# DarianNwankwo/Rollout-Bayesian-Optimization

Hardware: NVIDIA B200
Metric: rollout trajectories/sec (value+grad) (higher is better)
Workload: dtype f64

## Files before the change

### rollout-bayesian-optimization_b200/csrc/rollout_kernel.cu

```cuda
#include "rbo_kernel.cuh"

#ifndef RBO_VGLOB
#define RBO_VGLOB 0
#endif
#if RBO_VGLOB
#define RBO_ROW_UNROLL _Pragma("unroll 4")
#else
#define RBO_ROW_UNROLL _Pragma("unroll 2")
#endif
#if RBO_VGLOB
#define RBO_KERNEL_NAME rbo_rollout_kernel_largen
#define g_phase_cycles g_phase_cycles_largen
#define g_aux_cycles g_aux_cycles_largen
#define g_tr_cycles g_tr_cycles_largen
#else
#define RBO_KERNEL_NAME rbo_rollout_kernel
#endif

namespace rbo {

#ifdef RBO_PHASE_TIMERS
__device__ unsigned long long g_phase_cycles[16];
__device__ unsigned long long g_aux_cycles[16];
__device__ unsigned long long g_tr_cycles[16];
#define TR_T(v) long long v = clock64()
#define TR_ADD(i, t0, t1) do { if ((threadIdx.x & 31) == 0) atomicAdd(&g_tr_cycles[i], (unsigned long long)((t1) - (t0))); } while (0)
#define AUX_T(v) long long v = clock64()
#define AUX_ADD(i, t0) do { } while (0)
#define PT_DECL long long pt_t0 = clock64()
#define PT_MARK(i) do { if (threadIdx.x == 0) { long long t1_ = clock64(); atomicAdd(&g_phase_cycles[i], (unsigned long long)(t1_ - pt_t0)); pt_t0 = t1_; } } while (0)
#else
#define PT_DECL
#define PT_MARK(i)
#define AUX_T(v)
#define AUX_ADD(i, t0)
#define TR_T(v)
#define TR_ADD(i, t0, t1)
#endif

namespace {

enum { I_M = 0, I_NACT = 1, I_TSTATUS = 2, I_BEST = 3, I_EVALS = 4, I_T = 5, I_CASE = 6, I_NEXT = 7, I_ARR = 64 };
constexpr unsigned FULL = 0xffffffffu;
#ifndef RBO_SPIN_CAP
#define RBO_SPIN_CAP (1u << 28)
#endif

__device__ __forceinline__ double warp_sum(double v) {
#pragma unroll
  for (int off = 16; off > 0; off >>= 1) v += __shfl_xor_sync(FULL, v, off);
  return v;
}
__device__ __forceinline__ double warp_max(double v) {
#pragma unroll
  for (int off = 16; off > 0; off >>= 1) v = fmax(v, __shfl_xor_sync(FULL, v, off));
  return v;
}
__device__ __forceinline__ double warp_min(double v) {
#pragma unroll
  for (int off = 16; off > 0; off >>= 1) v = fmin(v, __shfl_xor_sync(FULL, v, off));
  return v;
}
__device__ __forceinline__ double warp_max_nonneg(double v) {
  const unsigned hi = (unsigned)__double2hiint(v), lo = (unsigned)__double2loint(v);
  const unsigned mh = __reduce_max_sync(FULL, hi);
  const unsigned ml = __reduce_max_sync(FULL, hi == mh ? lo : 0u);
  return __hiloint2double((int)mh, (int)ml);
}
__device__ __forceinline__ int tri_idx(int p, int q, int n) { return p * n - (p * (p - 1)) / 2 + (q - p); }

__device__ __forceinline__ void dmma(double& c0, double& c1, double a, double b) {
  asm volatile("mma.sync.aligned.m8n8k4.row.col.f64.f64.f64.f64 {%0,%1}, {%2}, {%3}, {%0,%1};" : "+d"(c0), "+d"(c1) : "d"(a), "d"(b));
}
__device__ __forceinline__ void c_to_b(double c0, double c1, int g, int tg, double& b0, double& b1) {
    const int s0 = tg * 4 + (g >> 1), s1 = s0 + 16;
    const double a0 = __shfl_sync(FULL, c0, s0), a1 = __shfl_sync(FULL, c1, s0);
    const double e0 = __shfl_sync(FULL, c0, s1), e1 = __shfl_sync(FULL, c1, s1);
    b0 = (g & 1) ? a1 : a0; b1 = (g & 1) ? e1 : e0;
  }
__device__ __forceinline__ void fan_wbot(const double* V, const double* Fp, int RP, int N8, int cB, int nfan, int g, int tg, double& w0, double& w1) {
    const double t0 = (tg < nfan) ? V[(size_t)(N8 + tg) * RP + cB] : 0.0;
    const double t1 = (tg + 4 < nfan) ? V[(size_t)(N8 + tg + 4) * RP + cB] : 0.0;
    w0 = 0.0; w1 = 0.0;
    dmma(w0, w1, Fp[(size_t)(N8 + g) * 8 + tg], t0);
    dmma(w0, w1, Fp[(size_t)(N8 + g) * 8 + 4 + tg], t1);
    if (g >= nfan) { w0 = 0.0; w1 = 0.0; }
  }

__device__ __noinline__ void bwd_direct(double* V, const double* Fp, const int* colidx, const double* Lbf, int RP, int N8, int nb, int ncols, int nfan, int warp, int lane, double* scratch = nullptr) {
    const unsigned FULL = 0xffffffffu;
    const int g = lane >> 2, tg = lane & 3;
    const int ngroups = (ncols + 7) >> 3, ncls = (nb + 1) >> 1, tpg = ncls * 4;
    auto cols = [&](int group, int& cB, int& c0, int& c1, bool& v0, bool& v1) {
      const int i0 = 8 * group, first = colidx[i0];
      cB = (i0 + g < ncols) ? colidx[i0 + g] : first;
      v0 = i0 + 2 * tg < ncols; v1 = i0 + 2 * tg + 1 < ncols;
      c0 = v0 ? colidx[i0 + 2 * tg] : first; c1 = v1 ? colidx[i0 + 2 * tg + 1] : first;
    };
    if (nfan > 0) {
      const int ntile = N8 >> 3;
      for (int task = warp; task < ngroups * ntile; task += RBO_NWARPS) {
        const int group = task / ntile, i0 = 8 * (task - group * ntile);
        int cB, c0, c1; bool v0, v1;
        cols(group, cB, c0, c1, v0, v1);
        double w0, w1, b0, b1;
        fan_wbot(V, Fp, RP, N8, cB, nfan, g, tg, w0, w1);
        c_to_b(w0, w1, g, tg, b0, b1);
        double* vr = V + (size_t)(i0 + g) * RP;
        double x0 = vr[c0], x1 = vr[c1];
        dmma(x0, x1, Fp[(size_t)(i0 + g) * 8 + tg], -b0);
        dmma(x0, x1, Fp[(size_t)(i0 + g) * 8 + 4 + tg], -b1);
        __syncwarp();
        if (v0) vr[c0] = x0;
        if (v1) vr[c1] = x1;
      }
      __syncthreads();
      for (int group = warp; group < ngroups; group += RBO_NWARPS) {
        int cB, c0, c1; bool v0, v1;
        cols(group, cB, c0, c1, v0, v1);
        double w0, w1;
        fan_wbot(V, Fp, RP, N8, cB, nfan, g, tg, w0, w1);
        __syncwarp();
        if (v0) V[(size_t)(N8 + g) * RP + c0] = w0;
        if (v1) V[(size_t)(N8 + g) * RP + c1] = w1;
      }
    }
#if RBO_VGLOB
    {
      const int ntask = ngroups * ncls;
      __syncthreads();
      for (int task = warp; task < ntask; task += RBO_NWARPS) {
        const int group = task / ncls, cls = task - group * ncls;
        int cB, c0, c1; bool v0, v1;
        cols(group, cB, c0, c1, v0, v1);
        const int rp4 = 4 * RP, rp8 = 8 * RP;
        for (int hh = 0; hh < 2; ++hh) {
          const int ib = hh ? nb - 1 - cls : cls, rb = RBO_BR * ib;
          if (hh && ib == cls) continue;
          const int nc = nb - ib, chunk0 = nb * ib - ib * (ib - 1) / 2;
          const int nq = min(4, (N8 - rb + 7) >> 3);
          const double2* ap = reinterpret_cast<const double2*>(Lbf) + (size_t)chunk0 * 512 + lane;
          const double* vd = V + (size_t)(rb + tg) * RP + cB;
          double acc[4][4];
#pragma unroll
          for (int q = 0; q < 4; ++q) { acc[q][0] = acc[q][1] = acc[q][2] = acc[q][3] = 0.0; }
          for (int cc = 0; cc < nc; ++cc) {
            const double* v = (cc < nc - 1) ? vd + (size_t)(RBO_BR + RBO_CHUNK_K * cc) * RP : vd;
            double bv[8];
#pragma unroll
            for (int pp = 0; pp < 4; ++pp) { bv[2 * pp] = v[pp * rp8]; bv[2 * pp + 1] = v[pp * rp8 + rp4]; }
            const double2* ac = ap + (size_t)512 * cc;
#pragma unroll
            for (int q = 0; q < 4; ++q) {
              if (q < nq) {
                double2 A[4];
#pragma unroll
                for (int pp = 0; pp < 4; ++pp) A[pp] = __ldg(ac + 128 * q + 32 * pp);
#pragma unroll
                for (int pp = 0; pp < 4; ++pp) {
                  dmma(acc[q][0], acc[q][1], A[pp].x, bv[2 * pp]);
                  dmma(acc[q][2], acc[q][3], A[pp].y, bv[2 * pp + 1]);
                }
              }
            }
          }
#pragma unroll
          for (int q = 0; q < 4; ++q) {
            const int row = rb + 8 * q + g;
            if (q < nq && row < N8) {
              double* o = scratch + ((size_t)group * N8 + row) * 8 + 2 * tg;
              o[0] = acc[q][0] + acc[q][2]; o[1] = acc[q][1] + acc[q][3];
            }
          }
        }
      }
      __syncthreads();
      for (int idx = threadIdx.x; idx < ngroups * N8 * 8; idx += RBO_THREADS) {
        const int group = idx / (N8 * 8), r2 = idx - group * N8 * 8, row = r2 >> 3, cc = r2 & 7;
        if (8 * group + cc < ncols) V[(size_t)row * RP + colidx[8 * group + cc]] = scratch[idx];
      }
    }
#else
    const int gpb = RBO_NWARPS / tpg;
    for (int gb = 0; gb < ngroups; gb += gpb) {
      const int group = gb + warp / tpg, rem = warp % tpg, cls = rem >> 2, rq = rem & 3;
      const bool wact = warp < gpb * tpg && group < ngroups;
      int cB = 0, c0 = 0, c1 = 0; bool v0 = false, v1 = false;
      if (wact) cols(group, cB, c0, c1, v0, v1);
      double acc[2][2] = {{0.0, 0.0}, {0.0, 0.0}};
      const int rp4 = 4 * RP, rp8 = 8 * RP;
      __syncthreads();
#pragma unroll
      for (int hh = 0; hh < 2; ++hh) {
        const int ib = hh ? nb - 1 - cls : cls, rb = RBO_BR * ib;
        if (!wact || (hh && ib == cls) || rb + 8 * rq >= N8) continue;
// ... 817 lines not shown
      double* fv = V + cB;
      const int fp = tg;

      AUX_T(tf0_);
      if (!FWD && nfan > 0 && wact) {
        if (rq == 0) {
          double t[8], wb[8];
#pragma unroll
          for (int r = 0; r < 8; ++r) t[r] = (r < nfan) ? fv[(size_t)(N8 + r) * RP] : 0.0;
          __syncwarp();
#pragma unroll
          for (int r = 0; r < 8; ++r) {
            double s = 0.0;
#pragma unroll
            for (int kk = 0; kk < 8; ++kk) s = fma(Fp[(size_t)(N8 + r) * 8 + kk], t[kk], s);
            wb[r] = (r < nfan) ? s : 0.0;
          }
          if (vB && fp == 0) {
#pragma unroll
            for (int r = 0; r < 8; ++r) fv[(size_t)(N8 + r) * RP] = wb[r];
          }
          for (int i = fp; i < N8; i += 4) {
            const double* f = Fp + (size_t)i * 8;
            double s = 0.0;
#pragma unroll
            for (int r = 0; r < 8; ++r) s = fma(f[r], wb[r], s);
            if (vB) fv[(size_t)i * RP] -= s;
          }
        }
        group_sync(NRQ, gl);
      }

      AUX_ADD(1, tf0_);
      AUX_T(tc0_);
      double c[MTW][2];
#pragma unroll
      for (int mt = 0; mt < MTW; ++mt) { c[mt][0] = 0.0; c[mt][1] = 0.0; }
      const int rofs = 8 * MTW * rq;
      for (int i = 0; i < nb; ++i) {
        const int ib = FWD ? nb - 1 - i : i, nc = FWD ? ib + 1 : nb - ib, rb = RBO_BR * ib;
        for (int cc = 0; cc < nc; ++cc, ++q) {
#ifdef RBO_PHASE_TIMERS
          long long tw0 = clock64();
#endif
          full_wait(q);
#ifdef RBO_PHASE_TIMERS
          if (tid == 0) atomicAdd(&g_phase_cycles[FWD ? 12 : 13], (unsigned long long)(clock64() - tw0));
#endif
          const double* buf = stage + (size_t)(q % RBO_NSTAGE) * RBO_CHUNK_K * RBO_LP + rofs;
          AUX_T(tm0_);
          if (wact) {
            const int nt = (N8 - rb - rofs + 7) >> 3;
            if (cc < nc - 1) {
              const int krow0 = (FWD ? 0 : rb + RBO_BR) + cc * RBO_CHUNK_K;
              mma_chunk<MTW>(buf, V + (size_t)krow0 * RP, cB, g, tg, c, nt);
            } else {
              mma_chunk<MTW>(buf, V + (size_t)rb * RP, cB, g, tg, c, nt);
              AUX_T(td0_);
              group_sync(NRQ, gl);
#pragma unroll
              for (int mt = 0; mt < MTW; ++mt) {
                const int row = rb + rofs + 8 * mt + g;
                if (row < N8) {
                  if (v0) V[(size_t)row * RP + c0] = c[mt][0];
                  if (v1) V[(size_t)row * RP + c1] = c[mt][1];
                }
                c[mt][0] = 0.0; c[mt][1] = 0.0;
              }
              asm volatile("" ::: "memory");
              AUX_ADD(4, td0_);
            }
          }
          __syncwarp();
          AUX_ADD(3, tm0_);
          if (lane == 0) empty_arrive(q);
        }
      }

      AUX_ADD(2, tc0_);
      if (FWD && nfan > 0 && wact && NRQ > 1) group_sync(NRQ, gl);
      if (FWD && nfan > 0 && wact && rq == 0) {
        double a0[2] = {0.0, 0.0}, a1[2] = {0.0, 0.0};
        const double* fa = Fp + (size_t)tg * 8 + g;
        const double* vb = V + (size_t)tg * RP + cB;
        const int nkt = N8 >> 2;
#pragma unroll 2
        for (int kt = 0; kt < nkt; kt += 2) {
          dmma(a0[0], a1[0], fa[(size_t)(4 * kt) * 8], vb[(size_t)(4 * kt) * RP]);
          dmma(a0[1], a1[1], fa[(size_t)(4 * kt + 4) * 8], vb[(size_t)(4 * kt + 4) * RP]);
        }
        const double s0 = a0[0] + a0[1], s1 = a1[0] + a1[1];
        double* vr = V + (size_t)(N8 + g) * RP;
        const double t0 = (g < nfan) ? vr[c0] - s0 : 0.0, t1 = (g < nfan) ? vr[c1] - s1 : 0.0;
        double b0, b1, r0 = 0.0, r1 = 0.0;
        c_to_b(t0, t1, g, tg, b0, b1);
        dmma(r0, r1, Fp[(size_t)(N8 + tg) * 8 + g], b0);
        dmma(r0, r1, Fp[(size_t)(N8 + tg + 4) * 8 + g], b1);
        if (g >= nfan) { r0 = 0.0; r1 = 0.0; }
        __syncwarp();
        if (v0) vr[c0] = r0;
        if (v1) vr[c1] = r1;
        __syncwarp();
      }
    }
    qglob = q;
  }

  __device__ void assemble_warp(int sl, int aidx, int np, int RSpre, const double* p1, int nout1, int RS1, const double* pg, int noutg, int goff, int gld,
                                int RSg, int RShc, int RShw, double fstar, double* Href ) {
    const int d = P.d, dd = d * d, q1 = d + 1, T2 = d * (d + 1) / 2;
    const double* ppre = sm + pl.ppre; const double* phess = sm + pl.phess;
    const int nout_pre = np * q1;
    double* dmu = sm + pl.sdmu + sl * d; double* dsig = sm + pl.sdsig + sl * d; double* ga = sm + pl.sga + sl * d;
    double* Ht = sm + pl.sHt + sl * dd; double* gh = sm + pl.sgh + sl * 8;
    auto pre = [&](int e) {
      double s = 0.0;
      if (RSpre < 0) { for (int r = 0; r < RS1; ++r) s += p1[(size_t)r * nout1 + e * (-RSpre) + q1]; }
      else for (int r = 0; r < RSpre; ++r) s += ppre[(size_t)r * nout_pre + aidx * q1 + e];
      return s;
    };
    auto one = [&](int e) { double s = 0.0; for (int r = 0; r < RS1; ++r) s += p1[(size_t)r * nout1 + e]; return s; };
    auto gramf = [&](int p, int q) { double s = 0.0; for (int r = 0; r < RSg; ++r) s += pg[(size_t)r * noutg + goff + p * gld + q]; return s; };
    auto hes = [&](int which, int e) { double s = 0.0; const int RS = which ? RShw : RShc; for (int r = 0; r < RS; ++r) s += phess[((size_t)(r * np + aidx) * 2 + which) * (T2 + 1) + e]; return s; };
    const double mu = pre(0);
    const double var = P.k0 - one(0);
    const double sigma = sqrt(var), isg = 1.0 / sigma;
    const GPart g = rule_eval(P.rule_id, P.sigma_tol, mu, sigma, P.theta1, fstar);
    bool fin = isfinite(g.g);
    for (int p = lane; p < d; p += 32) {
      double m = pre(1 + p), sg = -one(1 + p) * isg;
      double a = g.g_mu * m + g.g_sig * sg;
      dmu[p] = m; dsig[p] = sg; ga[p] = a;
      fin = fin && isfinite(a);
    }
    __syncwarp();
    const double bC = hes(0, T2), bW = hes(1, T2);
    for (int e = lane; e < T2; e += 32) {
      const int pq = tbld[e], p = pq & 0xff, q = pq >> 8;
      double gram = gramf(p, q), hc = hes(0, e), hw = hes(1, e);
      if (p == q) { hc += bC; hw += bW; }
      double hs = (-dsig[p] * dsig[q] - gram - hw) * isg;
      double href = g.g_mumu * dmu[p] * dmu[q] + g.g_mu * hc + g.g_sigsig * dsig[p] * dsig[q] + g.g_sig * hs;
      double htrue = href + g.g_musig * (dmu[p] * dsig[q] + dsig[p] * dmu[q]);
      if (Href) { Href[p * d + q] = href; Href[q * d + p] = href; }
      Ht[p * d + q] = -htrue; Ht[q * d + p] = -htrue;
      fin = fin && isfinite(htrue);
    }
    fin = __all_sync(FULL, fin);
    if (lane == 0) {
      gh[0] = g.g; gh[1] = g.g_mu; gh[2] = g.g_sig; gh[3] = g.g_muth; gh[4] = g.g_sigth; gh[5] = sigma; gh[6] = mu;
      gh[7] = fin ? 1.0 : 0.0;
    }
    __syncwarp();
  }

  __device__ bool chol_warp(double* A, int n) const {
    for (int j = 0; j < n; ++j) {
      double t = 0.0;
      if (lane >= j && lane < n) {
        t = A[lane * n + j];
        for (int k = 0; k < j; ++k) t = fma(-A[lane * n + k], A[j * n + k], t);
      }
      const double tj = __shfl_sync(FULL, t, j);
      if (!(tj > 0.0) || !isfinite(tj)) return false;
      const double inv = rsqrt(tj);
      if (lane == j) A[j * n + j] = inv;
      else if (lane > j && lane < n) A[lane * n + j] = t * inv;
      __syncwarp();
    }
    return true;
  }

  __device__ bool slot_logic_warp(int sl, bool single = false) {
    const int d = P.d, dd = d * d;
    const rbo_solver_opts& o = P.so;
    double* x = sm + pl.sx + sl * d; double* xt = sm + pl.sxt + sl * d; double* g = sm + pl.sg + sl * d;
    double* H = sm + pl.sH + sl * dd;
    double* Ht = sm + pl.sHt + sl * dd;
    double* A = Ht;
    const double* ga = sm + pl.sga + sl * d; const double* gh = sm + pl.sgh + sl * 8;
    int* fr = sfr + 32 * sl;
    TR_T(l0_);
    double f = (sm + pl.sf)[sl], Delta = (sm + pl.slam)[sl], pred = (sm + pl.spred)[sl], alpha = (sm + pl.shs)[sl];
    int iters = siter[sl], tries = stry[sl], flg = sflag[sl];
    double sn = (sm + pl.ssn)[sl];
    const double at = gh[0];
    bool fin = gh[7] != 0.0;
    const int ph = phase[sl];
    __syncwarp();
    auto store = [&](int status, bool keep) {
      if (lane == 0) {
        (sm + pl.sf)[sl] = f; (sm + pl.slam)[sl] = Delta; (sm + pl.spred)[sl] = pred; (sm + pl.shs)[sl] = alpha; (sm + pl.ssn)[sl] = sn;
        siter[sl] = iters; stry[sl] = tries; sflag[sl] = flg;
        if (!keep) sstat[sl] = status;
        phase[sl] = keep ? 1 : 2;
      }
      __syncwarp();
      return keep;
    };
    const double* lb = sm + pl.sbnd; const double* ub = lb + d;
    const int T2 = d * (d + 1) / 2;
    auto accept_state = [&](double fnew) {
      alpha = at;
      f = fnew;
      if (flg & 1) {
        const double ia = 1.0 / at;
        for (int a = lane; a < d; a += 32) { x[a] = xt[a]; g[a] = -ga[a] * ia; }
        __syncwarp();
        for (int e = lane; e < T2; e += 32) {
          const int pq = tbld[e], p = pq & 0xff, q = pq >> 8;
          const double hv = Ht[p * d + q] * ia + g[p] * g[q];
          H[p * d + q] = hv; H[q * d + p] = hv;
        }
      } else {
        for (int a = lane; a < d; a += 32) { x[a] = xt[a]; g[a] = -ga[a]; }
        for (int i = lane; i < dd; i += 32) H[i] = Ht[i];
      }
      __syncwarp();
    };
    if (lane == 0) sevals[sl] += 1;
    bool fresh;
    if (ph == 0) {
      if (!fin) {
        for (int a = lane; a < d; a += 32) x[a] = xt[a];
        alpha = nan("");
        return store(RBO_SOLVE_NAN, false);
      }
      flg = (P.rule_id != RBO_RULE_LCB && at > 0.0) ? 1 : 0;
      accept_state((flg & 1) ? -log(at) : -at);
      if (single) return store(RBO_SOLVE_CONVERGED, false);
      double wmax = 0.0;
      for (int a = 0; a < d; ++a) wmax = fmax(wmax, P.ubs[a] - P.lbs[a]);
      Delta = fmin(o.delta0_box * wmax, o.delta0_ell * P.kern.th[0]);
      iters = 0; tries = 0;
      fresh = true;
    } else {
      fin = fin && (!(flg & 1) || at > 0.0);
      const double ft = fin ? ((flg & 1) ? -log(at) : -at) : 0.0;
      const double rho = fin ? (f - ft) / pred : -1.0;
      if (fin && rho >= o.eta) {
        accept_state(ft);
        if (rho > 0.75 && (flg & 2) && sn >= 0.8 * Delta) {
          double dm2 = 0.0;
          for (int a = 0; a < d; ++a) { const double wd = P.ubs[a] - P.lbs[a]; dm2 = fma(wd, wd, dm2); }
          Delta = fmin(2.0 * Delta, sqrt(dm2));
        } else if (rho < 0.25) Delta = 0.25 * sn;
        tries = 0;
        iters += 1;
        if (iters >= o.maxit) return store(RBO_SOLVE_MAXIT, false);
        fresh = true;
      } else {
        Delta = 0.25 * fmin(Delta, sn);
        tries += 1;
        if (tries >= o.maxtry) return store(RBO_SOLVE_STALLED, false);
        fresh = false;
      }
    }
    const bool in = lane < d;
    const double xa = in ? x[lane] : 0.0, gg = in ? g[lane] : 0.0;
    const double lba = in ? lb[lane] : 0.0, uba = in ? ub[lane] : 0.0;
    const bool act = in && ((xa <= lba && gg > 0.0) || (xa >= uba && gg < 0.0));
    const bool isfree = in && !act;
    const unsigned fmask = __ballot_sync(FULL, isfree);
    const int nfree = __popc(fmask);
    if (isfree) fr[__popc(fmask & ((1u << lane) - 1u))] = lane;
    double pg = warp_max_nonneg(isfree ? fabs(gg) : 0.0);
    if (flg & 1) pg *= alpha;
    __syncwarp();
    if (fresh && pg <= o.gtol * fmax(1.0, fabs(alpha))) return store(RBO_SOLVE_CONVERGED, false);
    const int myc = lane < nfree ? fr[lane] : 0;
    const double xmax = warp_max_nonneg(fabs(xa));
    for (;;) {
      double* yv = sm + pl.sdmu + sl * d;
      TR_T(l1_); TR_ADD(1, l0_, l1_); TR_ADD(0, 0, 1);
      const bool hit = (nfree >= 2 && nfree <= 16) ? tr_step16(H, g, fr, nfree, d, Delta, sm + pl.sdsig + sl * d, sm + pl.sga + sl * d, yv)
                                                  : tr_step_warp(H, g, fr, nfree, d, Delta, A, yv);
      const double t = lane < nfree ? yv[lane] : 0.0;
      TR_T(l2_); TR_ADD(2, l1_, l2_);
      if (in) xt[lane] = xa;
      __syncwarp();
      if (lane < nfree) xt[myc] = fmin(fmax(x[myc] + t, lb[myc]), ub[myc]);
      __syncwarp();
      const double sa = in ? xt[lane] - xa : 0.0;
      const double smax = warp_max_nonneg(fabs(sa));
      if (smax <= o.xtol * fmax(1.0, xmax)) { sn = sqrt(warp_sum(sa * sa)); return store(RBO_SOLVE_STEP_TINY, false); }
      if (in) yv[lane] = sa;
      __syncwarp();
      double hsv = 0.0;
      if (in) {
        const double* Hr = H + lane * d;
        if ((d & 1) == 0) {
          double h1 = 0.0;
          for (int b = 0; b < d; b += 2) {
            const double2 hh = *reinterpret_cast<const double2*>(Hr + b), ss = *reinterpret_cast<const double2*>(yv + b);
            hsv = fma(hh.x, ss.x, hsv); h1 = fma(hh.y, ss.y, h1);
          }
          hsv += h1;
        } else for (int b = 0; b < d; ++b) hsv = fma(Hr[b], yv[b], hsv);
      }
      double r0 = sa * sa, r1 = gg * sa, r2 = sa * hsv;
#pragma unroll
      for (int off = 16; off > 0; off >>= 1) {
        r0 += __shfl_xor_sync(FULL, r0, off); r1 += __shfl_xor_sync(FULL, r1, off); r2 += __shfl_xor_sync(FULL, r2, off);
      }
      sn = sqrt(r0);
      const double gs = r1, sHs = r2;
      const double pr = -(gs + 0.5 * sHs);
      if (!(pr > 0.0)) {
        Delta = 0.25 * fmin(Delta, sn);
        tries += 1;
        if (tries >= o.maxtry) return store(RBO_SOLVE_STALLED, false);
        continue;
      }
      const bool pred_tiny = pr <= o.pred_tol * fmax(1.0, fabs(f));
      if (!hit && (pred_tiny || smax <= o.stol * fmax(1.0, xmax))) {
        for (int a = lane; a < d; a += 32) x[a] = xt[a];
        alpha = (flg & 1) ? alpha * exp(pr) : alpha + pr;
        return store(RBO_SOLVE_FINAL_STEP, false);
      }
      if (pred_tiny) return store(RBO_SOLVE_PRED_TINY, false);
      pred = pr;
      flg = (flg & 1) | (hit ? 2 : 0);
      TR_T(l3_); TR_ADD(3, l2_, l3_);
      return store(0, true);
    }
  }

  __device__ void load_start(int sl, int sid) {
    const int d = P.d;
    phase[sl] = 0; sstat[sl] = RBO_SOLVE_MAXIT; siter[sl] = 0; stry[sl] = 0; sevals[sl] = 0; sstart[sl] = sid; sflag[sl] = 0;
    for (int a = 0; a < d; ++a) {
      double v = __ldg(P.starts + (size_t)sid * d + a);
      (sm + pl.sxt)[sl * d + a] = fmin(fmax(v, P.lbs[a]), P.ubs[a]);
    }
  }

  __device__ void multistart(size_t tape_off, bool single = false, bool first = false) {
    const int d = P.d, W = P.W, q1 = d + 1;
    __syncthreads();
    const unsigned short* evsrc = first ? evfirst : evprev;
    for (int i = tid; i < P.S; i += RBO_THREADS) {
      const unsigned e = evsrc[i];
      int r = 0;
      for (int j = 0; j < P.S; ++j) { const unsigned ej = evsrc[j]; r += (ej > e || (ej == e && j < i)) ? 1 : 0; }
      sorder[r] = (unsigned short)i;
    }
    __syncthreads();
    if (tid == 0) {
      si[I_BEST] = -1; si[I_EVALS] = 0; misc[0] = 0.0;
      const int n0 = single ? 1 : min(W, P.S);
      for (int i = 0; i < n0; ++i) { alist[i] = i; load_start(i, single ? i : (int)sorder[i]); }
      if (single) for (int a = 0; a < d; ++a) (sm + pl.sxt)[a] = bestx[a];
      si[I_NACT] = n0; si[I_NEXT] = single ? P.S : n0;
    }
    __syncthreads();
    int nact = si[I_NACT];
    PT_DECL;
    const long long round_cap = (long long)P.S * (P.so.maxit + 2) * (P.so.maxtry + 2);
    long long rounds_ = 0;
    while (nact > 0) {
      if (++rounds_ > round_cap) { if (tid == 0) P.work_counter[2] = 1; break; }
      auto pt = [&](int s) { return (const double*)(sm + pl.sxt + alist[s] * d); };
      auto cb = [&](int s) { return alist[s] * P.CS; };
      PT_MARK(9);
      fill_columns(nact, pt, cb);
      for (int i = tid; i < nact * q1; i += RBO_THREADS) { int s = i / q1; colidx[i] = alist[s] * P.CS + (i - s * q1); }
      const int nbq = nblk16(q1);
      __syncthreads();
      PT_MARK(0);
      tri_solve<true>(nact * q1, nf);
      const int q2 = q1 + 1;
      for (int s = tid; s < nact; s += RBO_THREADS) set_item(s, alist[s] * P.CS, q1, alist[s] * P.CS, q2, s * q1 * q2, UCOL);
      __syncthreads();
      PT_MARK(2);
      const int RS1 = choose_rs(nact * nbq * nblk16(q2)), RSg = RS1;
      colprod(nact, nact * q1 * q2, sm + pl.ppost, RS1);
      for (int i = tid; i < nact; i += RBO_THREADS) colidx[i] = alist[i] * P.CS;
      __syncthreads();
      PT_MARK(3);
      tri_solve<false>(nact, nf);
      __syncthreads();
      PT_MARK(4);
      const int nbd = nblk16(d);
      const int RShw = max(1, min(P.RSh, RBO_NWARPS / (nact * (nbd * (nbd + 1) / 2)))), RShc = RShw;
      hess_sums<3>(nact, pt, cb, cb, RShw);
      __syncthreads();
      PT_MARK(5);
      {
        const int n1 = nact * q1 * q2, nh = nact * 2 * (d * (d + 1) / 2 + 1);
        double* pp = sm + pl.ppost; double* ph = sm + pl.phess;
        if (RS1 > 1) for (int i = tid; i < n1; i += RBO_THREADS) { double a_ = pp[i]; for (int r = 1; r < RS1; ++r) a_ += pp[(size_t)r * n1 + i]; pp[i] = a_; }
        if (RShw > 1) for (int i = tid; i < nh; i += RBO_THREADS) { double a_ = ph[i]; for (int r = 1; r < RShw; ++r) a_ += ph[(size_t)r * nh + i]; ph[i] = a_; }
        __syncthreads();
      }
      for (int s = warp; s < nact; s += RBO_NWARPS) {
        const int sl = alist[s];
        assemble_warp(sl, s, nact, -q2, sm + pl.ppost + s * q1 * q2, nact * q1 * q2, 1, sm + pl.ppost, nact * q1 * q2, s * q1 * q2 + q2 + 1, q2, 1, 1, 1, misc[1], single ? sm + pl.sHref : nullptr);
#ifdef RBO_PHASE_TIMERS
        long long ta_ = clock64();
        if (tid == 0) atomicAdd(&g_phase_cycles[8], (unsigned long long)(ta_ - pt_t0));
#endif
        slot_logic_warp(sl, single);
#ifdef RBO_PHASE_TIMERS
        if (tid == 0) atomicAdd(&g_phase_cycles[14], (unsigned long long)(clock64() - ta_));
        if (lane == 0) { long long dt_ = clock64() - ta_; int b_ = (int)(dt_ / 4000); atomicAdd(&g_aux_cycles[b_ > 15 ? 15 : b_], 1ull); }
#endif
      }
      __syncthreads();
      PT_MARK(6);
      if (tid == 0) {
        int na2 = 0;
        for (int i = 0; i < nact; ++i) {
          const int sl = alist[i];
          if (phase[sl] == 1) { alist[na2++] = sl; continue; }
          const int sid = sstart[sl];
          const double f = -(sm + pl.shs)[sl];
          const double* x = sm + pl.sx + sl * d;
          bool bad = !isfinite(f);
          for (int a = 0; a < d; ++a) bad = bad || isnan(x[a]);
          si[I_EVALS] += sevals[sl];
          if (!single) { evprev[sid] = (unsigned short)min(sevals[sl], 65535); if (first) evfirst[sid] = evprev[sid]; }
          if (P.start_status && !single) P.start_status[tape_off + sid] = sstat[sl];
          if (P.start_iters && !single) P.start_iters[tape_off + sid] = siter[sl];
          if (!bad && (si[I_BEST] < 0 || f < misc[0] || (f == misc[0] && sid < si[I_BEST]))) {
            si[I_BEST] = sid; misc[0] = f;
            for (int a = 0; a < d; ++a) bestx[a] = x[a];
          }
          if (si[I_NEXT] < P.S) { load_start(sl, (int)sorder[si[I_NEXT]]); si[I_NEXT] += 1; alist[na2++] = sl; }
        }
        si[I_NACT] = na2;
      }
      __syncthreads();
      PT_MARK(7);
#ifdef RBO_PHASE_TIMERS
      if (tid == 0) atomicAdd(&g_phase_cycles[15], 1ull);
#endif
      nact = si[I_NACT];
    }
    if (tid == 0 && si[I_BEST] < 0) {
      if (si[I_TSTATUS] == RBO_TRAJ_OK) si[I_TSTATUS] = RBO_TRAJ_ALL_STARTS_NAN;
      for (int a = 0; a < d; ++a) bestx[a] = nan("");
    }
    __syncthreads();
  }
};

}

__global__ void __launch_bounds__(RBO_THREADS, 1) RBO_KERNEL_NAME(const __grid_constant__ DevProblem P) {
  extern __shared__ __align__(128) double smem[];
  K k(P, smem);
  const int tid = k.tid, d = P.d, N8 = P.N8, NR = P.NR, RP = P.RP, h = P.h, q1 = d + 1;
  double* bestx = k.bestx;
  double* misc = k.misc;
  int* si = k.si;
  k.build_tables();
  for (int i = tid; i < 2 * d; i += RBO_THREADS) smem[P.pl.sbnd + i] = i < d ? P.lbs[i] : P.ubs[i - d];
  for (int i = tid; i < P.S; i += RBO_THREADS) { k.evprev[i] = 0; k.evfirst[i] = 0; }
  k.pipe_init();
  for (int i = tid; i < NR * RP; i += RBO_THREADS) k.V[i] = 0.0;
  if (P.xsm) for (int i = tid; i < d * N8; i += RBO_THREADS) k.Xs[(i / N8) * P.XP + (i % N8)] = __ldg(P.Xb + i);
  __syncthreads();

  for (;;) {
    __syncthreads();
    if (tid == 0) {
      const int i = atomicAdd(P.work_counter, 1);
      si[I_M] = (i < P.M) ? (P.order ? P.order[i] : i) : P.M;
    }
    __syncthreads();
    const int m = si[I_M];
    if (m >= P.M) break;
#define RBO_MS (m % P.Ms)
#define RBO_MB (m / P.Ms)

    for (int i = tid; i < (N8 + RBO_MAXFAN) * 8; i += RBO_THREADS) k.Fp[i] = 0.0;
    for (int i = tid; i < 64; i += RBO_THREADS) k.G[i] = ((i >> 3) == (i & 7)) ? 1.0 : 0.0;
    for (int i = tid; i < NR; i += RBO_THREADS) { double c = (i < N8) ? __ldg(P.c0 + i) : 0.0; k.cst[i] = c; k.V[(size_t)i * RP + k.CCOL] = c; }
    for (int i = tid; i < NR; i += RBO_THREADS) { double u0 = (i < N8) ? __ldg(P.u0 + i) : 0.0; k.u[i] = u0; k.V[(size_t)i * RP + k.UCOL] = u0; }
    __syncthreads();
    if (tid < 8) k.Fp[(size_t)(N8 + tid) * 8 + tid] = 1.0;
    if (tid == 0) { misc[1] = P.ymin_base; si[I_TSTATUS] = RBO_TRAJ_OK; }
    k.nf = 0;
    __syncthreads();

    const bool myopic = (P.flags & RBO_FLAG_MYOPIC_INTERNAL) != 0;
    for (int step = myopic ? 1 : 0; step <= (myopic ? 1 : h); ++step) {
      if (step == 0) {
        if (tid < d) bestx[tid] = P.x0_batch ? __ldg(P.x0_batch + (size_t)RBO_MB * d + tid) : P.x0[tid];
        __syncthreads();
      } else {
        for (int pass = 0; pass < 2; ++pass) {
          const bool single = pass == 1;
          if (single && (myopic || !(P.flags & RBO_FLAG_TAPE_EX))) break;
          if (!single && !myopic && (P.flags & RBO_FLAG_TEACHER_FORCED)) {
            if (tid < d) bestx[tid] = (P.flags & RBO_FLAG_REPLAY_TAPE) ? P.xs[((size_t)m * (h + 1) + step) * d + tid] : P.x_forced[((size_t)RBO_MS * h + (step - 1)) * d + tid];
            if (tid == 0) { si[I_EVALS] = 0; misc[0] = nan(""); }
          } else {
            if (single) __syncthreads();
            k.multistart(single ? 0 : (myopic ? (size_t)m * P.S : ((size_t)m * h + (step - 1)) * P.S), single, !single && step == 1);
          }
          __syncthreads();
          if (!single) {
            if (!myopic && tid == 0) {
              if (P.n_evals) P.n_evals[(size_t)m * h + step - 1] = si[I_EVALS];
              if (P.alphas) P.alphas[(size_t)m * h + step - 1] = -misc[0];
            }
          } else {
            const size_t o = (size_t)m * h + step - 1;
            const double* gh = smem + k.pl.sgh;
            if (tid == 0) { P.t_mu[o] = gh[6]; P.t_sigma[o] = gh[5]; if (P.alphas) P.alphas[o] = gh[0]; }
            for (int i = tid; i < d; i += RBO_THREADS) { P.t_dmu[o * d + i] = (smem + k.pl.sdmu)[i]; P.t_dsigma[o * d + i] = (smem + k.pl.sdsig)[i]; }
            for (int i = tid; i < d * d; i += RBO_THREADS) P.t_Halpha[o * d * d + i] = (smem + k.pl.sHref)[i];
            __syncthreads();
          }
        }
      }
      if (myopic) {
        if (tid < d) P.xs[(size_t)m * d + tid] = bestx[tid];
        if (tid == 0) {
          P.values[m] = -misc[0];
          if (P.n_evals) P.n_evals[m] = si[I_EVALS];
          if (P.status) P.status[m] = si[I_TSTATUS];
          if (P.best_index) P.best_index[m] = si[I_BEST];
          if (P.grad_case) P.grad_case[m] = 0;
        }
        break;
      }

      {
        PT_DECL;
        auto pt = [&](int) { return (const double*)bestx; };
        auto cb0 = [&](int) { return 0; };
        k.fill_columns(1, pt, cb0);
        k.set_column(k.UCOL, k.u);
        for (int i = tid; i < q1; i += RBO_THREADS) k.colidx[i] = i;
        if (tid == 0) k.set_item(0, 0, q1, k.CCOL, 1, 0);
        __syncthreads();
        const int nbq = K::nblk16(q1);
        const int RSpre = k.choose_rs(nbq);
        k.colprod(1, q1, smem + k.pl.ppre, RSpre);
        __syncthreads();
        k.tri_solve<true>(q1, k.nf);
        if (tid == 0) { k.set_item(0, 0, q1, 0, q1, 0); k.set_item(1, 0, 1, k.UCOL, 1, q1 * q1); }
        __syncthreads();
        const int nsg = q1 * q1 + 1;
        const int RSpost = k.choose_rs(nbq * nbq + 1);
        k.colprod(2, nsg, smem + k.pl.ppost, RSpost);
        __syncthreads();
        double* Sg = misc + 8;
        for (int e = tid; e < nsg; e += RBO_THREADS) {
          double acc = 0.0;
          for (int r = 0; r < RSpost; ++r) acc += (smem + k.pl.ppost)[(size_t)r * nsg + e];
          if (e < q1 * q1) {
            const int p = e / q1, q = e - p * q1;
            const double dk = (p == q) ? (p == 0 ? P.k0 : -P.d2k0) : 0.0;
            if (p <= q) { Sg[p * q1 + q] = dk - acc; Sg[q * q1 + p] = dk - acc; }
            if (p == 0) misc[8 + q1 * q1 + q1 + q] = acc;
            if (e == 0) misc[4] = acc;
          } else misc[5] = acc;
        }
        if (tid < q1) {
          double acc = 0.0;
          for (int r = 0; r < RSpre; ++r) acc += (smem + k.pl.ppre)[(size_t)r * q1 + tid];
          misc[8 + q1 * q1 + tid] = acc;
        }
        __syncthreads();
        if (tid == 0) {
          const int r = k.nf;
          const double* dmu = misc + 8 + q1 * q1;
          double yv;
          if (P.flags & RBO_FLAG_GAUSS_HERMITE) {
            const double* raw = misc + 8 + q1 * q1 + q1;
            const double var = P.k0 - raw[0];
            if (!(var >= 0.0) && si[I_TSTATUS] == RBO_TRAJ_OK) si[I_TSTATUS] = RBO_TRAJ_NEG_VARIANCE;
            const double sigma = sqrt(var), node = __ldg(P.gh_nodes + (size_t)RBO_MS * P.gh_depth + step), s2n = 1.4142135623730951 * node;
            yv = dmu[0] + s2n * sigma;
            for (int a = 0; a < d; ++a) k.gyf[r * d + a] = dmu[1 + a] + s2n * (-raw[1 + a] / sigma);
          } else {
            bool pd = chol_inplace(Sg, q1, q1);
            if (!pd && si[I_TSTATUS] == RBO_TRAJ_OK) si[I_TSTATUS] = RBO_TRAJ_NOT_PD_JOINT;
            const double* rnm = P.rn + (size_t)RBO_MS + (size_t)P.Ms * q1 * step;
            yv = dmu[0] + Sg[0] * __ldg(rnm);
            for (int a = 0; a < d; ++a) {
              double v = dmu[1 + a];
              for (int j = 0; j <= a + 1; ++j) v += Sg[(a + 1) * q1 + j] * __ldg(rnm + (size_t)P.Ms * j);
              k.gyf[r * d + a] = v;
            }
          }
          k.yf[r] = yv;
          for (int a = 0; a < d; ++a) k.Xf[r * d + a] = bestx[a];
          misc[1] = fmin(misc[1], yv);
          double s = (P.k0 + P.sigma_n2) - misc[4];
          if (!(s > 0.0) && si[I_TSTATUS] == RBO_TRAJ_OK) si[I_TSTATUS] = RBO_TRAJ_NOT_PD_ROW;
          double lrr = sqrt(s);
          for (int j = 0; j < r; ++j) k.G[r * 8 + j] = k.V[(size_t)(N8 + j) * RP];
          k.G[r * 8 + r] = lrr;
          for (int cc = 0; cc < 8; ++cc) {
            double col[8];
            for (int rr = 0; rr < 8; ++rr) {
              double t = (rr == cc) ? 1.0 : 0.0;
              for (int j = cc; j < rr; ++j) t -= k.G[rr * 8 + j] * col[j];
              col[rr] = (rr < cc) ? 0.0 : t / k.G[rr * 8 + rr];
            }
            for (int rr = 0; rr < 8; ++rr) k.Fp[(size_t)(N8 + cc) * 8 + rr] = col[rr];
          }
          k.u[N8 + r] = (yv - misc[5]) / lrr;
          k.V[(size_t)(N8 + r) * RP + k.UCOL] = k.u[N8 + r];
        }
        __syncthreads();
        {
          const int r = k.nf;
          for (int j = tid; j < N8; j += RBO_THREADS) k.Fp[(size_t)j * 8 + r] = k.V[(size_t)j * RP];
          for (int j = tid; j < NR; j += RBO_THREADS) k.V[(size_t)j * RP + k.CCOL] = k.u[j];
          if (tid == 0) k.colidx[0] = k.CCOL;
        }
        k.nf += 1;
        __syncthreads();
        k.tri_solve<false>(1, k.nf);
        __syncthreads();
        for (int j = tid; j < NR; j += RBO_THREADS) k.cst[(size_t)(step + 1) * NR + j] = k.V[(size_t)j * RP + k.CCOL];
        __syncthreads();
        PT_MARK(10);
      }
    }

    if (myopic) continue;
    if (tid == 0) {
      double best = k.yf[0];
      int t = 0;
      for (int j = 1; j <= h; ++j) if (k.yf[j] < best) { best = k.yf[j]; t = j; }
      double val = fmax(P.fmini - best, 0.0);
      if (P.flags & RBO_FLAG_GAUSS_HERMITE) {
        const double* wq = P.gh_weights + (size_t)RBO_MS * P.gh_depth;
        val = __ldg(wq + t) * val / 1.7724538509055159;
        for (int j = 0; j <= h; ++j)
          for (int a = 0; a < d; ++a) k.gyf[j * d + a] *= __ldg(wq + j);
      }
      P.values[m] = val;
      si[I_T] = t;
      int tc = 0;
      if (P.mode == RBO_MODE_VALUE_GRAD) tc = (P.fmini <= best) ? 1 : (t == 0 ? 2 : 3);
      si[I_CASE] = tc;
      if (P.best_index) P.best_index[m] = t;
      if (P.grad_case) P.grad_case[m] = tc;
    }
    __syncthreads();
    if (P.xs) for (int i = tid; i < (h + 1) * d; i += RBO_THREADS) P.xs[(size_t)m * (h + 1) * d + i] = k.Xf[i];
    if (P.gys) for (int i = tid; i < (h + 1) * d; i += RBO_THREADS) P.gys[(size_t)m * (h + 1) * d + i] = k.gyf[i];
    if (P.ys) for (int i = tid; i <= h; i += RBO_THREADS) P.ys[(size_t)m * (h + 1) + i] = k.yf[i];
    __syncthreads();

    PT_DECL;
    if (P.mode == RBO_MODE_VALUE_GRAD) {
      const int tc = si[I_CASE], t = si[I_T], nth = P.ntheta;
      if (tc == 1) {
        for (int i = tid; i < d; i += RBO_THREADS) P.grad_x[(size_t)m * d + i] = 0.0;
        for (int i = tid; i < nth; i += RBO_THREADS) P.grad_theta[(size_t)m * nth + i] = 0.0;
      } else if (tc == 2) {
        for (int i = tid; i < d; i += RBO_THREADS) P.grad_x[(size_t)m * d + i] = -k.gyf[i];
        for (int i = tid; i < nth; i += RBO_THREADS) P.grad_theta[(size_t)m * nth + i] = 0.0;
      } else {
        double* xbars = k.adj; double* accr = k.adj + 9 * d; double* ybars = k.adj + 18 * d; double* gxa = ybars + 12; double* gtha = gxa + d;
        for (int i = tid; i < 19 * d + 16; i += RBO_THREADS) k.adj[i] = 0.0;
        __syncthreads();
        if (tid == 0) ybars[t + 1] = 1.0;
        const int CB_RAW = 0, CB_SOL = d + 3, CB_U = 2 * d + 4, CB_Q = 3 * d + 5;
        const double* dd_m = P.dual_dirs ? P.dual_dirs + (size_t)RBO_MS * h * d : nullptr;
        for (int i = t; i >= 1; --i) {
          k.nf = i;
          const double* c = k.cst + (size_t)i * NR;
          const double* xi = k.Xf + (size_t)i * d;
          auto pt = [&](int) { return xi; };
          auto cbr = [&](int) { return CB_RAW; };
          auto cbs = [&](int) { return CB_SOL; };
          __syncthreads();
          k.fill_columns(1, pt, cbr);
          k.set_column(k.CCOL, c);
          __syncthreads();
          for (int idx = tid; idx < NR * q1; idx += RBO_THREADS) {
            int j = idx / q1, q = idx - j * q1;
            k.V[(size_t)j * RP + CB_SOL + q] = k.V[(size_t)j * RP + CB_RAW + q];
          }
          for (int q = tid; q < q1; q += RBO_THREADS) k.colidx[q] = CB_SOL + q;
          if (tid == 0) k.set_item(0, CB_RAW, q1, k.CCOL, 1, 0);
          __syncthreads();
          const int nbq = K::nblk16(q1), nbd = K::nblk16(d);
          const int RSpre = k.choose_rs(nbq);
          k.colprod(1, q1, smem + k.pl.ppre, RSpre);
          k.tri_solve<true>(q1, k.nf);
          __syncthreads();
          if (tid == 0) k.set_item(0, CB_SOL, q1, CB_SOL, q1, 0);
          __syncthreads();
          const int RSpost = k.choose_rs(nbq * nbq);
          k.colprod(1, q1 * q1, smem + k.pl.ppost, RSpost);
          __syncthreads();
          k.tri_solve<false>(q1, k.nf);
          __syncthreads();
          const int RShess = k.choose_rs(nbd * (nbd + 1) / 2);
          k.hess_sums<3>(1, pt, cbr, cbs, RShess);
          __syncthreads();
          if (k.warp == 0) {
            double fst = P.ymin_base;
            for (int j = 0; j < i; ++j) fst = fmin(fst, k.yf[j]);
            k.assemble_warp(0, 0, 1, RSpre, smem + k.pl.ppost, q1 * q1, RSpost, smem + k.pl.ppost, q1 * q1, q1 + 1, q1, RSpost, RShess, RShess, fst, smem + k.pl.sHref);
            if (tid == 0) {
              misc[2] = fst;
              double* Hlu = smem + k.pl.sHt;
              const double* Href = smem + k.pl.sHref;
              int piv[RBO_MAXD];
              double det;
              for (int a = 0; a < d; ++a) for (int b = 0; b < d; ++b) Hlu[a * d + b] = Href[a * d + b];
              lu_factor(Hlu, d, piv, &det);
              double* xb = xbars + (size_t)i * d;
              if (det < P.htol) {
                for (int a = 0; a < d; ++a) xb[a] = 0.0;
                misc[3] = 0.0;
              } else {
                for (int a = 0; a < d; ++a) xb[a] = -k.gyf[(size_t)(i - 1) * d + a] * ybars[i + 1] - accr[(size_t)i * d + a];
                for (int a = 0; a < d; ++a) for (int b = 0; b < d; ++b) Hlu[a * d + b] = Href[b * d + a];
                double det2;
                if (!lu_factor(Hlu, d, piv, &det2) && si[I_TSTATUS] == RBO_TRAJ_OK) si[I_TSTATUS] = RBO_TRAJ_SINGULAR_HESSIAN;
                lu_solve(Hlu, d, piv, xb);
                misc[3] = 1.0;
                const double* gh = smem + k.pl.sgh; const double* dmu = smem + k.pl.sdmu; const double* dsg = smem + k.pl.sdsig;
                double s = 0.0;
                for (int a = 0; a < d; ++a) s += (dmu[a] * gh[3] + dsg[a] * gh[4]) * xb[a];
                gtha[0] += s;
              }
            }
          }
          __syncthreads();
          if (misc[3] == 0.0) continue;
          const double* xb = xbars + (size_t)i * d;
          const double sigma = (smem + k.pl.sgh)[5];
          for (int p = 0; p < i; ++p) {
            const int rowp = N8 + p;
            const double* xp = k.Xf + (size_t)p * d;
            for (int j = tid; j < NR; j += RBO_THREADS) {
              double* rowU = k.V + (size_t)j * RP + CB_U; double* rowQ = k.V + (size_t)j * RP + CB_Q;
              if (!k.row_active(j) || j == rowp) { for (int q = 0; q < q1; ++q) { rowU[q] = 0.0; rowQ[q] = 0.0; } continue; }
              double rho2 = 0.0;
              for (int a = 0; a < d; ++a) { double r = k.xcoord(j, a) - xp[a]; rho2 = fma(r, r, rho2); }
              double psi, a_, b_, gb_;
              kern_radial(P.kern, rho2, psi, a_, b_, gb_);
              if (!(rho2 > 0.0)) b_ = 0.0;
              double cp = k.V[(size_t)rowp * RP + k.CCOL], rd = 0.0;
              for (int a = 0; a < d; ++a) {
                double r = k.xcoord(j, a) - xp[a];
                double uu = -b_ * r;
                rowU[a] = uu; rowQ[a] = uu * cp;
                if (dd_m) rd += r * dd_m[(size_t)p * d + a];
              }
              double ud = -b_ * rd;
              rowU[d] = ud; rowQ[d] = ud * cp;
            }
            if (tid == 0) { k.set_item(0, CB_U, q1, k.CCOL, 1, 0); k.set_item(1, CB_U, q1, CB_SOL, 1, q1); }
            __syncthreads();
            const int RSb = k.choose_rs(2 * nbq);
            k.colprod(2, 2 * q1, smem + k.pl.ppost, RSb);
            __syncthreads();
// ... 284 lines not shown
```

Baseline: 22110.

## Parallelize per-step joint Cholesky and start loading across warp/threads

Result: faster. 22470 (median of 6 runs) (+1.6%).

```diff
diff --git a/rollout-bayesian-optimization_b200/csrc/rollout_kernel.cu b/rollout-bayesian-optimization_b200/csrc/rollout_kernel.cu
--- a/rollout-bayesian-optimization_b200/csrc/rollout_kernel.cu
+++ b/rollout-bayesian-optimization_b200/csrc/rollout_kernel.cu
@@ -40,7 +40,7 @@
 
 namespace {
 
-enum { I_M = 0, I_NACT = 1, I_TSTATUS = 2, I_BEST = 3, I_EVALS = 4, I_T = 5, I_CASE = 6, I_NEXT = 7, I_ARR = 64 };
+enum { I_M = 0, I_NACT = 1, I_TSTATUS = 2, I_BEST = 3, I_EVALS = 4, I_T = 5, I_CASE = 6, I_NEXT = 7, I_LOAD = 16, I_ARR = 64 };
 constexpr unsigned FULL = 0xffffffffu;
 #ifndef RBO_SPIN_CAP
 #define RBO_SPIN_CAP (1u << 28)
@@ -1164,6 +1164,24 @@
       gh[7] = fin ? 1.0 : 0.0;
     }
     __syncwarp();
+  }
+
+  __device__ __noinline__ bool chol_warp_seq(double* A, int n) const {
+    for (int j = 0; j < n; ++j) {
+      double s = A[j * n + j];
+      for (int k = 0; k < j; ++k) s -= A[j * n + k] * A[j * n + k];
+      if (!(s > 0.0) || !isfinite(s)) return false;
+      const double ljj = sqrt(s);
+      __syncwarp();
+      if (lane == 0) A[j * n + j] = ljj;
+      for (int i = j + 1 + lane; i < n; i += 32) {
+        double t = A[i * n + j];
+        for (int k = 0; k < j; ++k) t -= A[i * n + k] * A[j * n + k];
+        A[i * n + j] = t / ljj;
+      }
+      __syncwarp();
+    }
+    return true;
   }
 
   __device__ bool chol_warp(double* A, int n) const {
@@ -1339,11 +1357,16 @@
   }
 
   __device__ void load_start(int sl, int sid) {
-    const int d = P.d;
     phase[sl] = 0; sstat[sl] = RBO_SOLVE_MAXIT; siter[sl] = 0; stry[sl] = 0; sevals[sl] = 0; sstart[sl] = sid; sflag[sl] = 0;
-    for (int a = 0; a < d; ++a) {
-      double v = __ldg(P.starts + (size_t)sid * d + a);
-      (sm + pl.sxt)[sl * d + a] = fmin(fmax(v, P.lbs[a]), P.ubs[a]);
+    const int n = si[I_LOAD];
+    si[I_LOAD + 1 + 2 * n] = sl; si[I_LOAD + 2 + 2 * n] = sid; si[I_LOAD] = n + 1;
+  }
+  __device__ void load_queued() {
+    const int d = P.d, n = si[I_LOAD];
+    const double* lb = sm + pl.sbnd;
+    for (int i = tid; i < n * d; i += RBO_THREADS) {
+      const int e = i / d, a = i - e * d, sl = si[I_LOAD + 1 + 2 * e], sid = si[I_LOAD + 2 + 2 * e];
+      (sm + pl.sxt)[sl * d + a] = fmin(fmax(__ldg(P.starts + (size_t)sid * d + a), lb[a]), lb[d + a]);
     }
   }
 
@@ -1359,13 +1382,14 @@
     }
     __syncthreads();
     if (tid == 0) {
-      si[I_BEST] = -1; si[I_EVALS] = 0; misc[0] = 0.0;
+      si[I_BEST] = -1; si[I_EVALS] = 0; misc[0] = 0.0; si[I_LOAD] = 0;
       const int n0 = single ? 1 : min(W, P.S);
       for (int i = 0; i < n0; ++i) { alist[i] = i; load_start(i, single ? i : (int)sorder[i]); }
-      if (single) for (int a = 0; a < d; ++a) (sm + pl.sxt)[a] = bestx[a];
+      if (single) { si[I_LOAD] = 0; for (int a = 0; a < d; ++a) (sm + pl.sxt)[a] = bestx[a]; }
       si[I_NACT] = n0; si[I_NEXT] = single ? P.S : n0;
     }
     __syncthreads();
+    if (si[I_LOAD] > 0) { load_queued(); __syncthreads(); }
     int nact = si[I_NACT];
     PT_DECL;
     const long long round_cap = (long long)P.S * (P.so.maxit + 2) * (P.so.maxtry + 2);
@@ -1422,6 +1446,7 @@
       PT_MARK(6);
       if (tid == 0) {
         int na2 = 0;
+        si[I_LOAD] = 0;
         for (int i = 0; i < nact; ++i) {
           const int sl = alist[i];
           if (phase[sl] == 1) { alist[na2++] = sl; continue; }
@@ -1443,9 +1468,10 @@
         si[I_NACT] = na2;
       }
       __syncthreads();
+      if (si[I_LOAD] > 0) { load_queued(); __syncthreads(); }
       PT_MARK(7);
 #ifdef RBO_PHASE_TIMERS
-      if (tid == 0) atomicAdd(&g_phase_cycles[15], 1ull);
+      if (tid == 0) { atomicAdd(&g_phase_cycles[15], 1ull); atomicAdd(&g_tr_cycles[10], (unsigned long long)nact); }
 #endif
       nact = si[I_NACT];
     }
@@ -1578,47 +1604,57 @@
           misc[8 + q1 * q1 + tid] = acc;
         }
         __syncthreads();
-        if (tid == 0) {
+        if (k.warp == 0) {
+          const int lane = k.lane;
           const int r = k.nf;
           const double* dmu = misc + 8 + q1 * q1;
-          double yv;
-          if (P.flags & RBO_FLAG_GAUSS_HERMITE) {
-            const double* raw = misc + 8 + q1 * q1 + q1;
-            const double var = P.k0 - raw[0];
-            if (!(var >= 0.0) && si[I_TSTATUS] == RBO_TRAJ_OK) si[I_TSTATUS] = RBO_TRAJ_NEG_VARIANCE;
-            const double sigma = sqrt(var), node = __ldg(P.gh_nodes + (size_t)RBO_MS * P.gh_depth + step), s2n = 1.4142135623730951 * node;
-            yv = dmu[0] + s2n * sigma;
-            for (int a = 0; a < d; ++a) k.gyf[r * d + a] = dmu[1 + a] + s2n * (-raw[1 + a] / sigma);
-          } else {
-            bool pd = chol_inplace(Sg, q1, q1);
-            if (!pd && si[I_TSTATUS] == RBO_TRAJ_OK) si[I_TSTATUS] = RBO_TRAJ_NOT_PD_JOINT;
+          double yv = 0.0;
+          if (!(P.flags & RBO_FLAG_GAUSS_HERMITE)) {
+            double* rnv = misc + 8 + q1 * q1 + 2 * q1;
             const double* rnm = P.rn + (size_t)RBO_MS + (size_t)P.Ms * q1 * step;
-            yv = dmu[0] + Sg[0] * __ldg(rnm);
-            for (int a = 0; a < d; ++a) {
+            for (int j = lane; j < q1; j += 32) rnv[j] = __ldg(rnm + (size_t)P.Ms * j);
+            __syncwarp();
+            const bool pd = k.chol_warp_seq(Sg, q1);
+            if (lane == 0) {
+              if (!pd && si[I_TSTATUS] == RBO_TRAJ_OK) si[I_TSTATUS] = RBO_TRAJ_NOT_PD_JOINT;
+              yv = dmu[0] + Sg[0] * rnv[0];
+            }
+            for (int a = lane; a < d; a += 32) {
               double v = dmu[1 + a];
-              for (int j = 0; j <= a + 1; ++j) v += Sg[(a + 1) * q1 + j] * __ldg(rnm + (size_t)P.Ms * j);
+              for (int j = 0; j <= a + 1; ++j) v += Sg[(a + 1) * q1 + j] * rnv[j];
               k.gyf[r * d + a] = v;
             }
           }
-          k.yf[r] = yv;
-          for (int a = 0; a < d; ++a) k.Xf[r * d + a] = bestx[a];
-          misc[1] = fmin(misc[1], yv);
-          double s = (P.k0 + P.sigma_n2) - misc[4];
-          if (!(s > 0.0) && si[I_TSTATUS] == RBO_TRAJ_OK) si[I_TSTATUS] = RBO_TRAJ_NOT_PD_ROW;
-          double lrr = sqrt(s);
-          for (int j = 0; j < r; ++j) k.G[r * 8 + j] = k.V[(size_t)(N8 + j) * RP];
-          k.G[r * 8 + r] = lrr;
-          for (int cc = 0; cc < 8; ++cc) {
-            double col[8];
+          for (int a = lane; a < d; a += 32) k.Xf[r * d + a] = bestx[a];
+          if (lane == 0) {
+            if (P.flags & RBO_FLAG_GAUSS_HERMITE) {
+              const double* raw = misc + 8 + q1 * q1 + q1;
+              const double var = P.k0 - raw[0];
+              if (!(var >= 0.0) && si[I_TSTATUS] == RBO_TRAJ_OK) si[I_TSTATUS] = RBO_TRAJ_NEG_VARIANCE;
+              const double sigma = sqrt(var), node = __ldg(P.gh_nodes + (size_t)RBO_MS * P.gh_depth + step), s2n = 1.4142135623730951 * node;
+              yv = dmu[0] + s2n * sigma;
+              for (int a = 0; a < d; ++a) k.gyf[r * d + a] = dmu[1 + a] + s2n * (-raw[1 + a] / sigma);
+            }
+            k.yf[r] = yv;
+            misc[1] = fmin(misc[1], yv);
+            double s = (P.k0 + P.sigma_n2) - misc[4];
+            if (!(s > 0.0) && si[I_TSTATUS] == RBO_TRAJ_OK) si[I_TSTATUS] = RBO_TRAJ_NOT_PD_ROW;
+            double lrr = sqrt(s);
+            for (int j = 0; j < r; ++j) k.G[r * 8 + j] = k.V[(size_t)(N8 + j) * RP];
+            k.G[r * 8 + r] = lrr;
+            k.u[N8 + r] = (yv - misc[5]) / lrr;
+            k.V[(size_t)(N8 + r) * RP + k.UCOL] = k.u[N8 + r];
+          }
+          __syncwarp();
+          if (lane < 8) {
+            const int cc = lane;
+            double* col = k.Fp + (size_t)(N8 + cc) * 8;
             for (int rr = 0; rr < 8; ++rr) {
               double t = (rr == cc) ? 1.0 : 0.0;
               for (int j = cc; j < rr; ++j) t -= k.G[rr * 8 + j] * col[j];
               col[rr] = (rr < cc) ? 0.0 : t / k.G[rr * 8 + rr];
             }
-            for (int rr = 0; rr < 8; ++rr) k.Fp[(size_t)(N8 + cc) * 8 + rr] = col[rr];
-          }
-          k.u[N8 + r] = (yv - misc[5]) / lrr;
-          k.V[(size_t)(N8 + r) * RP + k.UCOL] = k.u[N8 + r];
+          }
         }
         __syncthreads();
         {
```
